# fundamentalvision/BEVFormer

Measured on AMD Instinct MI355X. Metric: BEV-encoder queries/sec (200x200 BEV, 6 cams, 4 lvls), higher is better.
Workload: dtype f32/bf16x3; 1 GPU; bevformer_base BEV encoder forward, 1 frame/step, 200x200 queries, 6 cams, 4 levels, 6 layers, with history BEV; sca_row_order=image, global_batch=1, parallelism=single GPU

## Files before the change

### bevformer_amd/csrc/bevmsda_linear.hip

```cpp
#include "../../include/bevmsda.h"
#include "linear_mfma.h"
#include "linear_pipe.h"
#include "linear_panel.h"
#include "linear_chain.h"
#include "wgrad_mfma.h"
#include "wgrad_tr.h"

namespace {
constexpr bool kLinearPipeDefault = false;
constexpr long long kLinearPipeMaxRows = 8192;
constexpr long long kChainSmallRows = 8192;
inline bool misaligned(const void *p) { return (reinterpret_cast<uintptr_t>(p) & 15u) != 0; }
}

extern "C" {

static int linear_launch(const float *x0, const float *a0, const float *x1, const float *a1, const float *w,
                         const uint16_t *wpack, const float *bias, const bevmsda_linear_desc *d, float *y,
                         void *stream, const int32_t *gidx = nullptr, const float *gscale = nullptr,
                         const float *mask = nullptr, long ldmask = 0, float mask_scale = 1.0f) {
  if (!d) return BEVMSDA_ERR_NULL_POINTER;
  if (d->M < 0 || d->N < 0 || d->K0 < 0 || d->K1 < 0) return BEVMSDA_ERR_BAD_SHAPE;
  if (d->precision != 0 && d->precision != 1) return BEVMSDA_ERR_BAD_OPTION;
  if (d->M == 0 || d->N == 0) return BEVMSDA_OK;
  if (d->K0 == 0 || d->K0 % bevmsda::kLinKGran != 0 || d->K1 % bevmsda::kLinKGran != 0) return BEVMSDA_ERR_UNSUPPORTED;
  if (!x0 || (!w && !wpack) || !y || (d->K1 > 0 && !x1)) return BEVMSDA_ERR_NULL_POINTER;
  if (d->ldx0 % 4 != 0 || (w && d->ldw % 4 != 0) || (a0 && d->lda0 % 4 != 0) ||
      (d->K1 > 0 && (d->ldx1 % 4 != 0 || (a1 && d->lda1 % 4 != 0))))
    return BEVMSDA_ERR_UNSUPPORTED;
  const int gcols = d->group_cols;
  if (gcols < 0) return BEVMSDA_ERR_BAD_SHAPE;
  if (gcols > 0 && (gcols % bevmsda::kLinBN != 0 || d->N % gcols != 0)) return BEVMSDA_ERR_UNSUPPORTED;
  if (d->ldx0 < d->K0 || (w && d->ldw < d->K0 + d->K1) || d->ldy < (gcols > 0 ? gcols : d->N) ||
      (d->K1 > 0 && d->ldx1 < d->K1))
    return BEVMSDA_ERR_BAD_SHAPE;
  if (misaligned(x0) || (w && misaligned(w)) || (wpack && misaligned(wpack)) ||
      (reinterpret_cast<uintptr_t>(y) & 3u) != 0 || (a0 && misaligned(a0)) ||
      (d->K1 > 0 && (misaligned(x1) || (a1 && misaligned(a1)))))
    return BEVMSDA_ERR_MISALIGNED;
  bevmsda::LinArgs a;
  a.x0 = x0; a.a0 = a0; a.x1 = d->K1 > 0 ? x1 : nullptr; a.a1 = d->K1 > 0 ? a1 : nullptr;
  a.ldx0 = d->ldx0; a.lda0 = d->lda0; a.ldx1 = d->ldx1; a.lda1 = d->lda1;
  a.w = w; a.ldw = d->ldw; a.wpack = wpack; a.bias = bias; a.y = y; a.ldy = d->ldy;
  a.gidx = gidx; a.gscale = gscale;
  a.M = d->M; a.N = d->N; a.K0 = d->K0; a.K1 = d->K1; a.relu = d->relu ? 1 : 0;
  a.group_cols = gcols;
  a.out_bf16 = d->out_bf16 ? 1 : 0;
  a.accum = d->reserved[0] == 1 ? 1 : 0;
  if (d->reserved[0] != 0 && d->reserved[0] != 1) return BEVMSDA_ERR_BAD_OPTION;
  a.mask = mask; a.ldmask = ldmask; a.mask_scale = mask_scale;
  if (mask && (gcols != 0 || d->out_bf16 || d->N % 4 != 0 || d->ldy % 4 != 0 || ldmask % 4 != 0 || ldmask < d->N ||
               misaligned(y) || misaligned(mask) || (bias && misaligned(bias)) || d->variant == 131))
    return BEVMSDA_ERR_UNSUPPORTED;
  if (a.accum && (d->out_bf16 || d->N % 4 != 0 || d->ldy % 4 != 0 || gcols % 4 != 0 || misaligned(y) || (bias && misaligned(bias)) ||
                  d->variant == 131))
    return BEVMSDA_ERR_UNSUPPORTED;
  hipStream_t st = static_cast<hipStream_t>(stream);
  const bool add = a.a0 != nullptr || a.a1 != nullptr || gidx != nullptr;
  if (d->variant != 0 && d->variant != 1 && d->variant != 13 && d->variant != 131 && d->variant != 17) return BEVMSDA_ERR_BAD_OPTION;
  if (d->variant == 17) {
    if (!wpack || a.accum || mask || d->N <= 128 || d->N % 4 != 0 || d->ldy % 4 != 0 || misaligned(y) || (bias && misaligned(bias)))
      return BEVMSDA_ERR_UNSUPPORTED;
    const long long nbm = (d->M + 63) / 64, nbn = (d->N + 255) / 256;
    const long long grid = ((nbm + 7) / 8) * 8 * nbn;
    if (grid >= (1LL << 31) || nbm >= (1LL << 28)) return BEVMSDA_ERR_TOO_LARGE;
    a.nblk_m = static_cast<int>(nbm);
    a.nblk_n = static_cast<int>(nbn);
    const dim3 g(static_cast<unsigned>(grid)), b(256);
    if (d->precision == 0) {
      if (add) hipLaunchKernelGGL((bevmsda::linear_splitbf16_kernel<3, true, 32, true, 3, 256, false, 64>), g, b, 0, st, a);
      else hipLaunchKernelGGL((bevmsda::linear_splitbf16_kernel<3, false, 32, true, 3, 256, false, 64>), g, b, 0, st, a);
    } else {
      if (add) hipLaunchKernelGGL((bevmsda::linear_splitbf16_kernel<1, true, 32, true, 3, 256, false, 64>), g, b, 0, st, a);
      else hipLaunchKernelGGL((bevmsda::linear_splitbf16_kernel<1, false, 32, true, 3, 256, false, 64>), g, b, 0, st, a);
    }
    return hipGetLastError() == hipSuccess ? BEVMSDA_OK : BEVMSDA_ERR_LAUNCH;
  }
  {
    const int nch = (d->K0 + d->K1) / 32;
    const bool covered = wpack && !add && !a.accum && !mask && (d->N % 4) == 0 && (d->ldy % 4) == 0 && (gcols % 4) == 0 && !misaligned(y) &&
                         (!bias || !misaligned(bias)) && (!d->out_bf16 || (reinterpret_cast<uintptr_t>(y) & 7u) == 0) &&
                         (nch == 8 || nch == 16);
    if (d->variant == 131 && !covered) return BEVMSDA_ERR_UNSUPPORTED;
    if (covered && (d->variant == 131 || (d->variant == 0 && d->reserved[1] == 0 && (kLinearPipeDefault || d->M <= kLinearPipeMaxRows)))) {
      const long long nbm = (d->M + 127) / 128, nbn = (d->N + 127) / 128;
      const long long grid = ((nbm + 7) / 8) * 8 * nbn;
      if (grid >= (1LL << 31) || nbm >= (1LL << 28)) return BEVMSDA_ERR_TOO_LARGE;
      a.nblk_m = static_cast<int>(nbm);
      a.nblk_n = static_cast<int>(nbn);
#define BEVMSDA_PIPE(NP_, NCH_)                                                                                       \
  do {                                                                                                                \
    auto kern = bevmsda::linear_pipe_kernel<NP_, NCH_>;                                                               \
    const int dyn = 2 * ((NP_) == 3 ? 2 : 1) * bevmsda::kPipePlane * 2;                                               \
    if (hipFuncSetAttribute(reinterpret_cast<const void *>(kern), hipFuncAttributeMaxDynamicSharedMemorySize, dyn) != \
// ... 346 lines not shown
  do {                                                                                                                   \
    if (shape == 1 && deep && (PRE_) == 0)                                                                               \
      hipLaunchKernelGGL((bevmsda::linear_panel_kernel<NP_, 2, 2, 4, LN_, PRE_, 0, 0, false, 6>), grid, dim3(256), 0, st, a); \
    else if (shape == 1) hipLaunchKernelGGL((bevmsda::linear_panel_kernel<NP_, 2, 2, 4, LN_, PRE_>), grid, dim3(256), 0, st, a); \
    else hipLaunchKernelGGL((bevmsda::linear_panel_kernel<NP_, 4, 1, 8, LN_, PRE_>), grid, dim3(512), 0, st, a);           \
  } while (0)
#define BEVMSDA_PANEL(NP_, LN_)                              \
  do {                                                       \
    if (idx) BEVMSDA_PANEL2(NP_, LN_, 2);                    \
    else if (a.a0 || a.a1) BEVMSDA_PANEL2(NP_, LN_, 1);      \
    else BEVMSDA_PANEL2(NP_, LN_, 0);                        \
  } while (0)
  if (d->precision == 0) { if (ln) BEVMSDA_PANEL(3, true); else BEVMSDA_PANEL(3, false); }
  else { if (ln) BEVMSDA_PANEL(1, true); else BEVMSDA_PANEL(1, false); }
#undef BEVMSDA_PANEL2
#undef BEVMSDA_PANEL
  return hipGetLastError() == hipSuccess ? BEVMSDA_OK : BEVMSDA_ERR_LAUNCH;
}

int bevmsda_linear_panel_f32(const float *x0, const float *a0, const float *x1, const float *a1, const int32_t *idx,
                             const float *scale, const uint16_t *wpanel, const float *bias,
                             const bevmsda_linear_desc *d, const bevmsda_layernorm_desc *ln, float *y, void *stream) {
  return panel_launch(x0, a0, x1, a1, idx, scale, wpanel, bias, d, ln, y, stream, nullptr, 0, nullptr, 0);
}

int bevmsda_linear_panel_segments_f32(const float *x0, const uint16_t *wpanel, const float *bias, const bevmsda_linear_desc *d,
                                      const int32_t *seg_start, int64_t seg_len, const int64_t *level_shapes,
                                      int num_levels, float *y, void *stream) {
  if (!seg_start) return BEVMSDA_ERR_NULL_POINTER;
  return panel_launch(x0, nullptr, nullptr, nullptr, nullptr, nullptr, wpanel, bias, d, nullptr, y, stream, seg_start, seg_len,
                      level_shapes, num_levels);
}

int bevmsda_linear_panel_rows2_f32(const float *x_lo, const float *x_hi, int64_t m_split, const uint16_t *wpanel, const float *bias,
                                   const bevmsda_linear_desc *d, float *y, void *stream) {
  if (!x_hi) return BEVMSDA_ERR_NULL_POINTER;
  return panel_launch(x_lo, nullptr, nullptr, nullptr, nullptr, nullptr, wpanel, bias, d, nullptr, y, stream, nullptr, 0, nullptr, 0,
                      x_hi, m_split);
}

struct ChainTail {
  const float *first; long long ld_first;
  const float *pos; long long ld_pos;
  const uint16_t *w3p; const float *b3;
  float *proj; long long ld_proj;
  int n3;
};

static int ffn_chain_launch(const float *rows, const int32_t *idx, const float *scale, const uint16_t *w0p, const float *b0,
                            const float *res, const float *gamma0, const float *beta0, const uint16_t *w1p, const float *b1,
                            const uint16_t *w2p, const float *b2, const float *gamma1, const float *beta1,
                            const bevmsda_chain_desc *d, float *y, void *stream, bool save, float *sv_z0, float *sv_x,
                            float *sv_h, float *sv_z1, const float *dk0 = nullptr, const float *dkh = nullptr,
                            const float *dk1 = nullptr, const ChainTail *tp = nullptr) {
  if (!d) return BEVMSDA_ERR_NULL_POINTER;
  const bool drop = dk0 || dkh || dk1;
  if (tp) {
    if (save || drop) return BEVMSDA_ERR_BAD_OPTION;
    if (tp->n3 <= 0 || tp->n3 > 256 || tp->n3 % 64 != 0) return BEVMSDA_ERR_UNSUPPORTED;
    if (d->M > 0 && (!tp->first || !tp->w3p || !tp->proj)) return BEVMSDA_ERR_NULL_POINTER;
    if (tp->ld_first % 4 != 0 || tp->ld_proj % 4 != 0 || (tp->pos && tp->ld_pos % 4 != 0)) return BEVMSDA_ERR_UNSUPPORTED;
    if (tp->ld_first < 256 || tp->ld_proj < tp->n3 || (tp->pos && tp->ld_pos < 256)) return BEVMSDA_ERR_BAD_SHAPE;
    if (misaligned(tp->first) || misaligned(tp->w3p) || misaligned(tp->proj) || (tp->pos && misaligned(tp->pos)) ||
        (tp->b3 && misaligned(tp->b3)))
      return BEVMSDA_ERR_MISALIGNED;
  }
  if (drop && !save) return BEVMSDA_ERR_BAD_OPTION;
  if ((dk0 && misaligned(dk0)) || (dkh && misaligned(dkh)) || (dk1 && misaligned(dk1))) return BEVMSDA_ERR_MISALIGNED;
  if (save && d->M > 0 && (!sv_z0 || !sv_x || !sv_h || !sv_z1)) return BEVMSDA_ERR_NULL_POINTER;
  if (save && (misaligned(sv_z0) || misaligned(sv_x) || misaligned(sv_h) || misaligned(sv_z1))) return BEVMSDA_ERR_MISALIGNED;
  if (d->M < 0) return BEVMSDA_ERR_BAD_SHAPE;
  if (d->precision != 0 && d->precision != 1) return BEVMSDA_ERR_BAD_OPTION;
  if (d->C != bevmsda::kChainC || d->F != bevmsda::kChainF) return BEVMSDA_ERR_UNSUPPORTED;
  if (d->M == 0) return BEVMSDA_OK;
  if (!rows || !w0p || !w1p || !w2p || !gamma0 || !beta0 || !gamma1 || !beta1 || !y) return BEVMSDA_ERR_NULL_POINTER;
  if ((idx == nullptr) != (scale == nullptr)) return BEVMSDA_ERR_NULL_POINTER;
  if (d->ld_rows % 4 != 0 || d->ld_y % 4 != 0 || (res && d->ld_res % 4 != 0)) return BEVMSDA_ERR_UNSUPPORTED;
  if (d->ld_rows < d->C || d->ld_y < d->C || (res && d->ld_res < d->C)) return BEVMSDA_ERR_BAD_SHAPE;
  if (misaligned(rows) || misaligned(w0p) || misaligned(w1p) || misaligned(w2p) || misaligned(y) || (res && misaligned(res)) ||
      (b0 && misaligned(b0)) || (b1 && misaligned(b1)) || (b2 && misaligned(b2)) || misaligned(gamma0) || misaligned(beta0) ||
      misaligned(gamma1) || misaligned(beta1))
    return BEVMSDA_ERR_MISALIGNED;
  int shape = d->reserved[1];
  if (shape < 0 || shape > 3) return BEVMSDA_ERR_BAD_OPTION;
  const int gst = d->reserved[2] == 0 ? 2 : d->reserved[2];
  if (gst < 2 || gst > 64 || (gst > 2 && (!idx || save))) return BEVMSDA_ERR_BAD_OPTION;
  if (shape == 0) shape = (tp || d->M <= kChainSmallRows) ? 2 : (d->M >= 256LL * 64 ? 2 : 1);
  if (shape == 3) {
    const long long round64 = 256LL * 64;
    const long long head = (d->M / round64) * round64;
    const long long tail = d->M - head;
    if (head == 0 || tail == 0 || tail > 256LL * 2 * 32) {
      bevmsda_chain_desc one = *d;
      one.reserved[1] = (head == 0) ? 2 : 1;
      return ffn_chain_launch(rows, idx, scale, w0p, b0, res, gamma0, beta0, w1p, b1, w2p, b2, gamma1, beta1, &one, y, stream,
                              save, sv_z0, sv_x, sv_h, sv_z1, dk0, dkh, dk1, tp);
    }
    bevmsda_chain_desc dh = *d, dt = *d;
    dh.M = head; dh.reserved[1] = 1;
    dt.M = tail; dt.reserved[1] = 2;
    int rc = ffn_chain_launch(rows, idx, scale, w0p, b0, res, gamma0, beta0, w1p, b1, w2p, b2, gamma1, beta1, &dh, y, stream,
                              save, sv_z0, sv_x, sv_h, sv_z1, dk0, dkh, dk1, tp);
    if (rc != BEVMSDA_OK) return rc;
    const long long o = head;
    ChainTail tt{};
    if (tp) {
      tt = *tp;
      tt.first += o * tp->ld_first;
      if (tt.pos) tt.pos += o * tp->ld_pos;
      tt.proj += o * tp->ld_proj;
    }
    return ffn_chain_launch(idx ? rows : rows + o * d->ld_rows, idx ? idx + o * gst : nullptr, scale ? scale + o : nullptr, w0p, b0,
                            res ? res + o * d->ld_res : nullptr, gamma0, beta0, w1p, b1, w2p, b2, gamma1, beta1, &dt,
                            y + o * d->ld_y, stream, save, save ? sv_z0 + o * 256 : nullptr, save ? sv_x + o * 256 : nullptr,
                            save ? sv_h + o * 512 : nullptr, save ? sv_z1 + o * 256 : nullptr, dk0 ? dk0 + o * 256 : nullptr,
                            dkh ? dkh + o * 512 : nullptr, dk1 ? dk1 + o * 256 : nullptr, tp ? &tt : nullptr);
  }
  const int bm = shape == 1 ? 64 : 32;
  const long long nb = (d->M + bm - 1) / bm;
  if (nb >= (1LL << 31)) return BEVMSDA_ERR_TOO_LARGE;
  bevmsda::ChainArgs a{};
  a.rows = rows; a.ld_rows = d->ld_rows; a.gidx = idx; a.gscale = scale; a.gstride = gst;
  a.w0 = w0p; a.w1 = w1p; a.w2 = w2p; a.b0 = b0; a.b1 = b1; a.b2 = b2;
  a.res = res; a.ld_res = d->ld_res; a.gamma0 = gamma0; a.beta0 = beta0; a.gamma1 = gamma1; a.beta1 = beta1;
  a.eps0 = d->eps0; a.eps1 = d->eps1; a.y = y; a.ld_y = d->ld_y; a.M = d->M;
  a.sv_z0 = sv_z0; a.sv_x = sv_x; a.sv_h = sv_h; a.sv_z1 = sv_z1;
  a.dk0 = dk0; a.dkh = dkh; a.dk1 = dk1;
  if (tp) {
    a.tp_first = tp->first; a.ld_tp_first = tp->ld_first; a.tp_pos = tp->pos; a.ld_tp_pos = tp->ld_pos;
    a.w3 = tp->w3p; a.b3 = tp->b3; a.y3 = tp->proj; a.ld_y3 = tp->ld_proj; a.N3 = tp->n3;
  }
  hipStream_t st = static_cast<hipStream_t>(stream);
  const dim3 grid(static_cast<unsigned>(nb));
#define BEVMSDA_CHAIN_TP(NP_, PRE_)                                                                                               \
  do {                                                                                                                            \
    if (shape == 1) hipLaunchKernelGGL((bevmsda::linear_chain_kernel<NP_, PRE_, 0, 2, 1, 8, false, false, true>), grid, dim3(512), 0, st, a); \
    else hipLaunchKernelGGL((bevmsda::linear_chain_kernel<NP_, PRE_, 0, 1, 2, 4, false, false, true>), grid, dim3(256), 0, st, a);            \
  } while (0)
  if (tp) {
    if (d->precision == 0) { if (idx) BEVMSDA_CHAIN_TP(3, 2); else BEVMSDA_CHAIN_TP(3, 0); }
    else { if (idx) BEVMSDA_CHAIN_TP(1, 2); else BEVMSDA_CHAIN_TP(1, 0); }
    return hipGetLastError() == hipSuccess ? BEVMSDA_OK : BEVMSDA_ERR_LAUNCH;
  }
#undef BEVMSDA_CHAIN_TP
#define BEVMSDA_CHAIN(NP_, PRE_, SV_, DR_)                                                                                        \
  do {                                                                                                                            \
    if (shape == 1) hipLaunchKernelGGL((bevmsda::linear_chain_kernel<NP_, PRE_, 0, 2, 1, 8, SV_, DR_>), grid, dim3(512), 0, st, a); \
    else hipLaunchKernelGGL((bevmsda::linear_chain_kernel<NP_, PRE_, 0, 1, 2, 4, SV_, DR_>), grid, dim3(256), 0, st, a);            \
  } while (0)
  if (drop) {
    if (!idx) return BEVMSDA_ERR_UNSUPPORTED;
    if (d->precision == 0) BEVMSDA_CHAIN(3, 2, true, true); else BEVMSDA_CHAIN(1, 2, true, true);
  } else if (save) {
    if (d->precision == 0) { if (idx) BEVMSDA_CHAIN(3, 2, true, false); else BEVMSDA_CHAIN(3, 0, true, false); }
    else { if (idx) BEVMSDA_CHAIN(1, 2, true, false); else BEVMSDA_CHAIN(1, 0, true, false); }
  } else {
    if (d->precision == 0) { if (idx) BEVMSDA_CHAIN(3, 2, false, false); else BEVMSDA_CHAIN(3, 0, false, false); }
    else { if (idx) BEVMSDA_CHAIN(1, 2, false, false); else BEVMSDA_CHAIN(1, 0, false, false); }
  }
#undef BEVMSDA_CHAIN
  return hipGetLastError() == hipSuccess ? BEVMSDA_OK : BEVMSDA_ERR_LAUNCH;
}

int bevmsda_proj_ffn_chain_f32(const float *rows, const int32_t *idx, const float *scale, const uint16_t *w0p, const float *b0,
                               const float *res, const float *gamma0, const float *beta0, const uint16_t *w1p, const float *b1,
                               const uint16_t *w2p, const float *b2, const float *gamma1, const float *beta1,
                               const bevmsda_chain_desc *d, float *y, void *stream) {
  return ffn_chain_launch(rows, idx, scale, w0p, b0, res, gamma0, beta0, w1p, b1, w2p, b2, gamma1, beta1, d, y, stream, false,
                          nullptr, nullptr, nullptr, nullptr);
}
// ... 32 lines not shown
  if (d->M == 0) return BEVMSDA_OK;
  if (!grad_y || !save_z0 || !save_h || !save_z1 || !gamma0 || !gamma1 || !w0t_p || !w1t_p || !w2t_p || !grad_z1 || !grad_h ||
      !grad_z0 || !grad_in || !grad_gamma_beta1 || !grad_gamma_beta0)
    return BEVMSDA_ERR_NULL_POINTER;
  if (ld_grad_y % 4 != 0) return BEVMSDA_ERR_UNSUPPORTED;
  if (ld_grad_y < d->C) return BEVMSDA_ERR_BAD_SHAPE;
  if (misaligned(grad_y) || misaligned(save_z0) || misaligned(save_h) || misaligned(save_z1) || misaligned(gamma0) ||
      misaligned(gamma1) || misaligned(w0t_p) || misaligned(w1t_p) || misaligned(w2t_p) || misaligned(grad_z1) ||
      misaligned(grad_h) || misaligned(grad_z0) || misaligned(grad_in) || (reinterpret_cast<uintptr_t>(grad_gamma_beta1) & 3u) ||
      (reinterpret_cast<uintptr_t>(grad_gamma_beta0) & 3u))
    return BEVMSDA_ERR_MISALIGNED;
  const long long nb = (d->M + 31) / 32;
  if (nb >= (1LL << 31)) return BEVMSDA_ERR_TOO_LARGE;
  bevmsda::ChainArgs a{};
  a.w0 = w0t_p; a.w1 = w2t_p; a.w2 = w1t_p;
  a.gamma0 = gamma0; a.gamma1 = gamma1; a.eps0 = d->eps0; a.eps1 = d->eps1; a.M = d->M;
  a.bw_gy = grad_y; a.bw_ld_gy = ld_grad_y; a.bw_z1 = save_z1; a.bw_h = save_h; a.bw_z0 = save_z0;
  a.bw_gz1 = grad_z1; a.bw_gh = grad_h; a.bw_gz0 = grad_z0; a.bw_din = grad_in;
  a.bw_dgb1 = grad_gamma_beta1; a.bw_dgb0 = grad_gamma_beta0;
  if (drop0 && !grad_zp) return BEVMSDA_ERR_NULL_POINTER;
  if ((drop0 && misaligned(drop0)) || (drop1 && misaligned(drop1)) || (grad_zp && misaligned(grad_zp))) return BEVMSDA_ERR_MISALIGNED;
  a.dk0 = drop0; a.dk1 = drop1; a.bw_hscale = hidden_scale; a.bw_gzp = grad_zp;
  hipStream_t st = static_cast<hipStream_t>(stream);
  const dim3 grid(static_cast<unsigned>(nb));
  if (d->precision == 0) hipLaunchKernelGGL((bevmsda::linear_chain_kernel<3, 0, 2, 1, 2, 4, false, false>), grid, dim3(256), 0, st, a);
  else hipLaunchKernelGGL((bevmsda::linear_chain_kernel<1, 0, 2, 1, 2, 4, false, false>), grid, dim3(256), 0, st, a);
  return hipGetLastError() == hipSuccess ? BEVMSDA_OK : BEVMSDA_ERR_LAUNCH;
}

int bevmsda_proj_ln_proj_chain_backward_f32(const float *grad_proj, int64_t ld_grad_proj, const float *grad_x, const float *save_z0,
                                            const float *gamma0, const uint16_t *w0t_p, const uint16_t *w1t_p,
                                            const bevmsda_chain_desc *d, float *grad_z0, float *grad_in, float *grad_gamma_beta0,
                                            const float *drop0, float *grad_zp, void *stream) {
  if (!d) return BEVMSDA_ERR_NULL_POINTER;
  if (d->M < 0) return BEVMSDA_ERR_BAD_SHAPE;
  if (d->precision != 0 && d->precision != 1) return BEVMSDA_ERR_BAD_OPTION;
  const int N2 = d->reserved[0];
  if (d->C != bevmsda::kChainC || N2 <= 0 || N2 % 256 != 0 || N2 > bevmsda::kChainMaxN2) return BEVMSDA_ERR_UNSUPPORTED;
  if (d->M == 0) return BEVMSDA_OK;
  if (!grad_proj || !save_z0 || !gamma0 || !w0t_p || !w1t_p || !grad_z0 || !grad_in || !grad_gamma_beta0) return BEVMSDA_ERR_NULL_POINTER;
  if (ld_grad_proj % 4 != 0) return BEVMSDA_ERR_UNSUPPORTED;
  if (ld_grad_proj < N2) return BEVMSDA_ERR_BAD_SHAPE;
  if (misaligned(grad_proj) || (grad_x && misaligned(grad_x)) || misaligned(save_z0) || misaligned(gamma0) || misaligned(w0t_p) ||
      misaligned(w1t_p) || misaligned(grad_z0) || misaligned(grad_in) || (reinterpret_cast<uintptr_t>(grad_gamma_beta0) & 3u))
    return BEVMSDA_ERR_MISALIGNED;
  const long long nb = (d->M + 31) / 32;
  if (nb >= (1LL << 31)) return BEVMSDA_ERR_TOO_LARGE;
  bevmsda::ChainArgs a{};
  a.w0 = w0t_p; a.w1 = w1t_p; a.N2 = N2;
  a.gamma0 = gamma0; a.eps0 = d->eps0; a.M = d->M;
  a.bw_gy = grad_proj; a.bw_ld_gy = ld_grad_proj; a.bw_z1 = grad_x; a.bw_z0 = save_z0;
  a.bw_gz0 = grad_z0; a.bw_din = grad_in; a.bw_dgb0 = grad_gamma_beta0;
  if (drop0 && !grad_zp) return BEVMSDA_ERR_NULL_POINTER;
  if ((drop0 && misaligned(drop0)) || (grad_zp && misaligned(grad_zp))) return BEVMSDA_ERR_MISALIGNED;
  a.dk0 = drop0; a.bw_gzp = grad_zp; a.bw_hscale = 1.f;
  hipStream_t st = static_cast<hipStream_t>(stream);
  const dim3 grid(static_cast<unsigned>(nb));
  if (d->precision == 0) hipLaunchKernelGGL((bevmsda::linear_chain_kernel<3, 0, 3, 1, 2, 4, false, false>), grid, dim3(256), 0, st, a);
  else hipLaunchKernelGGL((bevmsda::linear_chain_kernel<1, 0, 3, 1, 2, 4, false, false>), grid, dim3(256), 0, st, a);
  return hipGetLastError() == hipSuccess ? BEVMSDA_OK : BEVMSDA_ERR_LAUNCH;
}

static int ln_proj_chain_launch(const float *rows, const int32_t *idx, const float *scale, const uint16_t *w0p, const float *b0,
                                const float *res, const float *gamma0, const float *beta0, const uint16_t *w1p, const float *b1,
                                const bevmsda_chain_desc *d, float *x_out, float *proj_out, void *stream, bool save,
                                float *sv_z0, const float *dk0 = nullptr) {
  if (!d) return BEVMSDA_ERR_NULL_POINTER;
  if (dk0 && (!save || misaligned(dk0))) return BEVMSDA_ERR_BAD_OPTION;
  if (save && d->M > 0 && !sv_z0) return BEVMSDA_ERR_NULL_POINTER;
  if (save && misaligned(sv_z0)) return BEVMSDA_ERR_MISALIGNED;
  if (d->M < 0) return BEVMSDA_ERR_BAD_SHAPE;
  if (d->precision != 0 && d->precision != 1) return BEVMSDA_ERR_BAD_OPTION;
  const long ld_y2 = d->reserved[0];
  if (d->C != bevmsda::kChainC || d->F <= 0 || d->F % 32 != 0 || d->F > bevmsda::kChainMaxN2) return BEVMSDA_ERR_UNSUPPORTED;
  if (d->M == 0) return BEVMSDA_OK;
  if (!rows || !w0p || !w1p || !gamma0 || !beta0 || !x_out || !proj_out) return BEVMSDA_ERR_NULL_POINTER;
  if ((idx == nullptr) != (scale == nullptr)) return BEVMSDA_ERR_NULL_POINTER;
  if (d->ld_rows % 4 != 0 || d->ld_y % 4 != 0 || ld_y2 % 4 != 0 || (res && d->ld_res % 4 != 0)) return BEVMSDA_ERR_UNSUPPORTED;
  if (d->ld_rows < d->C || d->ld_y < d->C || ld_y2 < d->F || (res && d->ld_res < d->C)) return BEVMSDA_ERR_BAD_SHAPE;
  if (misaligned(rows) || misaligned(w0p) || misaligned(w1p) || misaligned(x_out) || misaligned(proj_out) || (res && misaligned(res)) ||
      (b0 && misaligned(b0)) || (b1 && misaligned(b1)) || misaligned(gamma0) || misaligned(beta0))
    return BEVMSDA_ERR_MISALIGNED;
  int shape = d->reserved[1];
  if (shape < 0 || shape > 3) return BEVMSDA_ERR_BAD_OPTION;
  if (shape == 0) shape = d->M <= kChainSmallRows ? 2 : (d->M >= 256LL * 64 ? 2 : 1);
  if (d->F % 64 != 0) shape = 1;
  if (shape == 3) {
    const long long round64 = 256LL * 64;
    const long long head = (d->M / round64) * round64;
    const long long tail = d->M - head;
    bevmsda_chain_desc dh = *d, dt = *d;
    if (head == 0 || tail == 0 || tail > 256LL * 2 * 32) {
      dh.reserved[1] = (head == 0) ? 2 : 1;
      return ln_proj_chain_launch(rows, idx, scale, w0p, b0, res, gamma0, beta0, w1p, b1, &dh, x_out, proj_out, stream, save, sv_z0,
                                  dk0);
    }
    dh.M = head; dh.reserved[1] = 1;
    dt.M = tail; dt.reserved[1] = 2;
    int rc = ln_proj_chain_launch(rows, idx, scale, w0p, b0, res, gamma0, beta0, w1p, b1, &dh, x_out, proj_out, stream, save, sv_z0,
                                  dk0);
    if (rc != BEVMSDA_OK) return rc;
    const long long o = head;
    return ln_proj_chain_launch(idx ? rows : rows + o * d->ld_rows, idx ? idx + o * 2 : nullptr, scale ? scale + o : nullptr, w0p,
                                b0, res ? res + o * d->ld_res : nullptr, gamma0, beta0, w1p, b1, &dt, x_out + o * d->ld_y,
                                proj_out + o * ld_y2, stream, save, save ? sv_z0 + o * 256 : nullptr,
                                dk0 ? dk0 + o * 256 : nullptr);
  }
  const int bm = shape == 1 ? 64 : 32;
  const long long nb = (d->M + bm - 1) / bm;
  if (nb >= (1LL << 31)) return BEVMSDA_ERR_TOO_LARGE;
  bevmsda::ChainArgs a{};
  a.rows = rows; a.ld_rows = d->ld_rows; a.gidx = idx; a.gscale = scale;
  a.w0 = w0p; a.w1 = w1p; a.w2 = nullptr; a.b0 = b0; a.b1 = b1; a.b2 = nullptr;
  a.res = res; a.ld_res = d->ld_res; a.gamma0 = gamma0; a.beta0 = beta0; a.gamma1 = a.beta1 = nullptr;
  a.eps0 = d->eps0; a.eps1 = 0.f; a.y = x_out; a.ld_y = d->ld_y; a.M = d->M; a.y2 = proj_out; a.ld_y2 = ld_y2; a.N2 = d->F;
  a.sv_z0 = sv_z0;
  a.dk0 = dk0;
  hipStream_t st = static_cast<hipStream_t>(stream);
  const dim3 grid(static_cast<unsigned>(nb));
#define BEVMSDA_CHAIN(NP_, PRE_, SV_, DR_)                                                                                        \
  do {                                                                                                                            \
    if (shape == 1) hipLaunchKernelGGL((bevmsda::linear_chain_kernel<NP_, PRE_, 1, 2, 1, 8, SV_, DR_>), grid, dim3(512), 0, st, a); \
    else hipLaunchKernelGGL((bevmsda::linear_chain_kernel<NP_, PRE_, 1, 1, 2, 4, SV_, DR_>), grid, dim3(256), 0, st, a);            \
  } while (0)
  if (save) {
    if (idx) return BEVMSDA_ERR_UNSUPPORTED;
    if (dk0) { if (d->precision == 0) BEVMSDA_CHAIN(3, 0, true, true); else BEVMSDA_CHAIN(1, 0, true, true); }
    else { if (d->precision == 0) BEVMSDA_CHAIN(3, 0, true, false); else BEVMSDA_CHAIN(1, 0, true, false); }
  } else {
    if (d->precision == 0) { if (idx) BEVMSDA_CHAIN(3, 2, false, false); else BEVMSDA_CHAIN(3, 0, false, false); }
    else { if (idx) BEVMSDA_CHAIN(1, 2, false, false); else BEVMSDA_CHAIN(1, 0, false, false); }
  }
#undef BEVMSDA_CHAIN
  return hipGetLastError() == hipSuccess ? BEVMSDA_OK : BEVMSDA_ERR_LAUNCH;
}

int bevmsda_proj_ln_proj_chain_f32(const float *rows, const int32_t *idx, const float *scale, const uint16_t *w0p, const float *b0,
                                   const float *res, const float *gamma0, const float *beta0, const uint16_t *w1p, const float *b1,
                                   const bevmsda_chain_desc *d, float *x_out, float *proj_out, void *stream) {
  return ln_proj_chain_launch(rows, idx, scale, w0p, b0, res, gamma0, beta0, w1p, b1, d, x_out, proj_out, stream, false, nullptr);
}

int bevmsda_proj_ln_proj_chain_train_f32(const float *rows, const uint16_t *w0p, const float *b0, const float *res,
                                         const float *gamma0, const float *beta0, const uint16_t *w1p, const float *b1,
                                         const bevmsda_chain_desc *d, float *x_out, float *proj_out, float *save_z0,
                                         const float *drop0, void *stream) {
  return ln_proj_chain_launch(rows, nullptr, nullptr, w0p, b0, res, gamma0, beta0, w1p, b1, d, x_out, proj_out, stream, true,
                              save_z0, drop0);
}

}
```

### bevformer_amd/csrc/linear_chain.h

```cpp
#pragma once
#include <type_traits>
#include "linear_panel.h"
#include "scalar_ops.h"

namespace bevmsda {

struct ChainArgs {
  const float *rows;
  long ld_rows;
  const int32_t *gidx;
  int gstride;
  const float *gscale;
  const uint16_t *w0, *w1, *w2;
  const float *b0, *b1, *b2;
  const float *res;
  long ld_res;
  const float *gamma0, *beta0, *gamma1, *beta1;
  float eps0, eps1;
  float *y;
  long ld_y;
  long M;
  float *y2;
  long ld_y2;
  int N2;
// ... 42 lines not shown

constexpr int kChainC = 256, kChainF = 512;
constexpr int kChainMaxN2 = 768;

template <int NPROD, int PRE, int MODE = 0, int MT = 2, int NT = 1, int NW = 8, bool SAVE = false, bool DROP = false, bool TP = false>
__global__ void __launch_bounds__(NW * 64) __attribute__((amdgpu_waves_per_eu(2, 2)))
linear_chain_kernel(const ChainArgs a) {
  static_assert(NPROD == 1 || NPROD == 3, "NPROD");
  static_assert(!TP || (MODE == 0 && !SAVE && !DROP), "TP: the inference form of MODE 0");
  static_assert(PRE == 0 || PRE == 2, "PRE: 0 plain rows, 2 two-row gather");
  static_assert(MODE < 2 || (MT == 1 && NT == 2 && PRE == 0 && !SAVE && !DROP), "MODE 2 / 3: 32-row workgroups of 4 wavefronts");
  static_assert(NW * NT == 8 && (MT == 1 || MT == 2) && (NT == 1 || NT == 2), "workgroup shape");
  constexpr bool LO = NPROD == 3;
  constexpr int NPL = LO ? 2 : 1;
  constexpr int BM = MT * 32;
  constexpr int NTHREADS = NW * 64;
  constexpr int BUF = (BM / 8) * 4 * 2048;
  constexpr int PPW = (BM / 8) * 4 / NW;
  constexpr int NCST = 4 * kChainC + kChainMaxN2 + 2 * kChainC;
  constexpr int NSTAT = MODE >= 2 ? 2 : 1;
  __shared__ __attribute__((aligned(16))) unsigned char lds[2 * BUF + NSTAT * NW * BM * 4 + NCST * 4];
  unsigned char *const buf0 = lds, *const buf1 = lds + BUF;
  float *const stat = reinterpret_cast<float *>(lds + 2 * BUF);
  float *const cst = stat + NSTAT * NW * BM;
  float *const c_g0 = cst, *const c_be0 = cst + 256, *const c_g1 = cst + 512, *const c_be1 = cst + 768;
  float *const c_b1 = cst + 1024, *const c_b0 = cst + 1024 + kChainMaxN2, *const c_b2 = c_b0 + 256;
  const int nb1 = MODE == 1 ? a.N2 : kChainF;

  const int tid = threadIdx.x;
  const int lane = tid & 63;
  const int wave = __builtin_amdgcn_readfirstlane(tid >> 6);
  const long m0 = static_cast<long>(blockIdx.x) * BM;
#ifdef BEVMSDA_CHAIN_PROF
  unsigned long long t_prev_ = __builtin_readcyclecounter();
#endif

  {
    const float4 z4 = make_float4(0.f, 0.f, 0.f, 0.f);
    for (int t4 = tid * 4; t4 < NCST; t4 += NTHREADS * 4) {
      const float *src = nullptr;
      if (t4 < 256) src = a.gamma0 + t4;
      else if (t4 < 512) src = MODE >= 2 ? nullptr : a.beta0 + (t4 - 256);
      else if (t4 < 768) src = (MODE == 0 || MODE == 2) ? a.gamma1 + (t4 - 512) : nullptr;
      else if (t4 < 1024) src = MODE == 0 ? a.beta1 + (t4 - 768) : nullptr;
      else if (TP && t4 >= 1024 + kChainF && t4 < 1024 + kChainMaxN2)
        src = (a.b3 && t4 - 1024 - kChainF < a.N3) ? a.b3 + (t4 - 1024 - kChainF) : nullptr;
      else if (t4 < 1024 + kChainMaxN2) src = (a.b1 && t4 - 1024 < nb1) ? a.b1 + (t4 - 1024) : nullptr;
      else if (t4 < 1024 + kChainMaxN2 + 256) src = a.b0 ? a.b0 + (t4 - 1024 - kChainMaxN2) : nullptr;
      else src = (MODE == 0 && a.b2) ? a.b2 + (t4 - 1024 - kChainMaxN2 - 256) : nullptr;
      *reinterpret_cast<float4 *>(cst + t4) = src ? *reinterpret_cast<const float4 *>(src) : z4;
    }
  }

  const int f_r = lane & 31, f_h = lane >> 5;
  const int f_q0 = ((f_r >> 2) & 1) | ((f_r >> 4) << 1);
  const int f_rl = ((f_r & 3) << 1) | ((f_r >> 3) & 1);
  const int f_x = f_r & 7;
  unsigned f_addr[4];
#pragma unroll
  for (int sc = 0; sc < 4; ++sc)
    f_addr[sc] = static_cast<unsigned>(f_q0 * 4 * 2048 + (f_rl * 8 + (((2 * sc + f_h) ^ f_x))) * 16);
  unsigned p_addr[NT][4];
#pragma unroll
  for (int j = 0; j < NT; ++j)
#pragma unroll
    for (int g = 0; g < 4; ++g) {
      const int line = NT * wave + j;
      p_addr[j][g] = static_cast<unsigned>((f_q0 * 4 + (line >> 1)) * 2048 + (f_rl * 8 + ((f_h + 2 * g) ^ f_x)) * 16 + (line & 1) * 8);
    }

  const int wlane = lane * 16;
  lin_f32x16 acc[MT][NT], xk[MT][NT], acc2[MODE != 1 ? MT : 1][MODE != 1 ? NT : 1];

#ifndef BEVMSDA_CHAIN_WD
#define BEVMSDA_CHAIN_WD 2
#endif
  constexpr int WD = BEVMSDA_CHAIN_WD;
  lin_bf16x8 wf[WD + 1][NT][NPL];
  auto wload = [&](__amdgpu_buffer_rsrc_t wrsrc, int tile, int nstep, int st, int sg) {
#pragma unroll
    for (int j = 0; j < NT; ++j)
#pragma unroll
      for (int pl = 0; pl < NPL; ++pl)
        wf[st][j][pl] = __builtin_bit_cast(lin_bf16x8, __builtin_amdgcn_raw_buffer_load_b128(
                                                         wrsrc, wlane, (((tile * NT + j) * nstep + sg) * 2 + pl) * 1024, 0));
  };
  auto wprefetch = [&](__amdgpu_buffer_rsrc_t wrsrc, int tile, int nstep, int sg0) {
#pragma unroll
    for (int k = 0; k < WD; ++k) wload(wrsrc, tile, nstep, k, sg0 + k);
  };
  auto gemm16 = [&](auto &c, const unsigned char *buf, __amdgpu_buffer_rsrc_t wrsrc, int tile, int nstep, int sg0) {
    lin_bf16x8 af[2][MT][NPL];
    auto aload = [&](int set, int s) {
      const unsigned base = f_addr[s & 3] + (s >> 2) * 2048;
#pragma unroll
      for (int i = 0; i < MT; ++i)
#pragma unroll
        for (int pl = 0; pl < NPL; ++pl)
          af[set][i][pl] = *reinterpret_cast<const lin_bf16x8 *>(buf + base + i * (4 * 4 * 2048) + pl * 1024);
    };
    aload(0, 0);
#pragma unroll
    for (int s = 0; s < 16; ++s) {
      if (s + WD < 16) wload(wrsrc, tile, nstep, (s + WD) % (WD + 1), sg0 + s + WD);
      if (s + 1 < 16) aload((s + 1) & 1, s + 1);
      __builtin_amdgcn_sched_barrier(0);
#pragma unroll
      for (int j = 0; j < NT; ++j)
#pragma unroll
        for (int i = 0; i < MT; ++i) {
          if constexpr (LO) {
            c[i][j] = __builtin_amdgcn_mfma_f32_32x32x16_bf16(wf[s % (WD + 1)][j][0], af[s & 1][i][1], c[i][j], 0, 0, 0);
            c[i][j] = __builtin_amdgcn_mfma_f32_32x32x16_bf16(wf[s % (WD + 1)][j][1], af[s & 1][i][0], c[i][j], 0, 0, 0);
          }
          c[i][j] = __builtin_amdgcn_mfma_f32_32x32x16_bf16(wf[s % (WD + 1)][j][0], af[s & 1][i][0], c[i][j], 0, 0, 0);
        }
      __builtin_amdgcn_sched_barrier(0);
    }
  };
  auto zero = [&](auto &c) {
#pragma unroll
    for (int i = 0; i < MT; ++i)
#pragma unroll
      for (int j = 0; j < NT; ++j)
#pragma unroll
        for (int r = 0; r < 16; ++r) c[i][j][r] = 0.f;
  };
  auto to_planes = [&](const auto &c, unsigned char *buf) {
#pragma unroll
    for (int i = 0; i < MT; ++i)
#pragma unroll
      for (int j = 0; j < NT; ++j)
#pragma unroll
        for (int g = 0; g < 4; ++g) {
          const float v0 = c[i][j][4 * g], v1 = c[i][j][4 * g + 1], v2 = c[i][j][4 * g + 2], v3 = c[i][j][4 * g + 3];
          uint2 hi, lo;
          hi.x = lin_pack2(v0, v1);
          hi.y = lin_pack2(v2, v3);
          unsigned char *dst = buf + p_addr[j][g] + i * (4 * 4 * 2048);
          *reinterpret_cast<uint2 *>(dst) = hi;
          if (LO) {
            lo.x = lin_pack2(v0 - __uint_as_float(hi.x << 16), v1 - __uint_as_float(hi.x & 0xffff0000u));
            lo.y = lin_pack2(v2 - __uint_as_float(hi.y << 16), v3 - __uint_as_float(hi.y & 0xffff0000u));
            *reinterpret_cast<uint2 *>(dst + 1024) = lo;
          }
        }
  };
  auto ncol = [&](int j) { return (NT * wave + j) * 32 + 4 * (lane >> 5); };
  auto layernorm = [&](auto &c, const float *gamma, const float *beta, float eps) {
    float mean[MT], rstd[MT];
#pragma unroll
    for (int i = 0; i < MT; ++i) {
      float sum = 0.f;
#pragma unroll
      for (int j = 0; j < NT; ++j)
#pragma unroll
        for (int r = 0; r < 16; ++r) sum += c[i][j][r];
      sum += __shfl_xor(sum, 32, 64);
      mean[i] = sum;
    }
    if (lane < 32) {
#pragma unroll
      for (int i = 0; i < MT; ++i) stat[wave * BM + i * 32 + lane] = mean[i];
    }
    __syncthreads();
#pragma unroll
    for (int i = 0; i < MT; ++i) {
      float t = 0.f;
// ... 588 lines not shown
```

Measured before the change: 10.14 million BEV queries/s.

## Add persistent row-streaming chain kernel with LDS-DMA weight ring for LN+proj

Adds a persistent linear_chain_rows kernel, with one block per CU, where each wave owns 16 rows held in registers. Weight chunks stream through a four-stage LDS ring using global_load_lds DMA, so the GEMM+LayerNorm(+FFN) chain runs without re-reading activations. The kernel becomes the default for the LN+projection chain when M is at least 32768 and nothing is saved; the FFN chain uses it only when shape 4 is requested explicitly. The trade-off is that all waves must load the full weight set in every pass and synchronize at a barrier per chunk, which could limit throughput compared with the tiled panel kernels. A debug L2-probe macro is also added to the older chain kernel.

```diff
diff --git a/bevformer_amd/csrc/bevmsda_linear.hip b/bevformer_amd/csrc/bevmsda_linear.hip
--- a/bevformer_amd/csrc/bevmsda_linear.hip
+++ b/bevformer_amd/csrc/bevmsda_linear.hip
@@ -3,6 +3,7 @@
 #include "linear_pipe.h"
 #include "linear_panel.h"
 #include "linear_chain.h"
+#include "linear_chain_rows.h"
 #include "wgrad_mfma.h"
 #include "wgrad_tr.h"
 
@@ -10,6 +11,23 @@
 constexpr bool kLinearPipeDefault = false;
 constexpr long long kLinearPipeMaxRows = 8192;
 constexpr long long kChainSmallRows = 8192;
+constexpr long long kChainRowsMinRows = 32768;
+inline int device_cus() {
+  static int cus[64] = {0};
+  int dev = 0;
+  if (hipGetDevice(&dev) != hipSuccess || dev < 0 || dev >= 64) return 256;
+  if (cus[dev] == 0) {
+    int n = 0;
+    if (hipDeviceGetAttribute(&n, hipDeviceAttributeMultiprocessorCount, dev) != hipSuccess || n <= 0) n = 256;
+    cus[dev] = n;
+  }
+  return cus[dev];
+}
+inline dim3 chain_rows_grid(long long M) {
+  const long long groups8 = ((M + 15) / 16 + 7) / 8;
+  const long long cus = device_cus();
+  return dim3(static_cast<unsigned>(groups8 < cus ? groups8 : cus));
+}
 inline bool misaligned(const void *p) { return (reinterpret_cast<uintptr_t>(p) & 15u) != 0; }
 }
 
@@ -522,10 +540,33 @@
       misaligned(gamma1) || misaligned(beta1))
     return BEVMSDA_ERR_MISALIGNED;
   int shape = d->reserved[1];
-  if (shape < 0 || shape > 3) return BEVMSDA_ERR_BAD_OPTION;
+  if (shape < 0 || shape > 4) return BEVMSDA_ERR_BAD_OPTION;
   const int gst = d->reserved[2] == 0 ? 2 : d->reserved[2];
   if (gst < 2 || gst > 64 || (gst > 2 && (!idx || save))) return BEVMSDA_ERR_BAD_OPTION;
+  if (shape == 4 && (save || drop)) return BEVMSDA_ERR_BAD_OPTION;
   if (shape == 0) shape = (tp || d->M <= kChainSmallRows) ? 2 : (d->M >= 256LL * 64 ? 2 : 1);
+  if (shape == 4) {
+    bevmsda::ChainArgs a{};
+    a.rows = rows; a.ld_rows = d->ld_rows; a.gidx = idx; a.gscale = scale; a.gstride = gst;
+    a.w0 = w0p; a.w1 = w1p; a.w2 = w2p; a.b0 = b0; a.b1 = b1; a.b2 = b2;
+    a.res = res; a.ld_res = d->ld_res; a.gamma0 = gamma0; a.beta0 = beta0; a.gamma1 = gamma1; a.beta1 = beta1;
+    a.eps0 = d->eps0; a.eps1 = d->eps1; a.y = y; a.ld_y = d->ld_y; a.M = d->M;
+    if (tp) {
+      a.tp_first = tp->first; a.ld_tp_first = tp->ld_first; a.tp_pos = tp->pos; a.ld_tp_pos = tp->ld_pos;
+      a.w3 = tp->w3p; a.b3 = tp->b3; a.y3 = tp->proj; a.ld_y3 = tp->ld_proj; a.N3 = tp->n3;
+    }
+    hipStream_t st = static_cast<hipStream_t>(stream);
+    const dim3 grid = chain_rows_grid(d->M);
+#define BEVMSDA_CHAIN_ROWS(NP_, TP_)                                                                                       \
+  do {                                                                                                                     \
+    if (idx) hipLaunchKernelGGL((bevmsda::linear_chain_rows_kernel<NP_, 2, 0, TP_>), grid, dim3(512), 0, st, a);          \
+    else hipLaunchKernelGGL((bevmsda::linear_chain_rows_kernel<NP_, 0, 0, TP_>), grid, dim3(512), 0, st, a);              \
+  } while (0)
+    if (tp) { if (d->precision == 0) BEVMSDA_CHAIN_ROWS(3, true); else BEVMSDA_CHAIN_ROWS(1, true); }
+    else { if (d->precision == 0) BEVMSDA_CHAIN_ROWS(3, false); else BEVMSDA_CHAIN_ROWS(1, false); }
+#undef BEVMSDA_CHAIN_ROWS
+    return hipGetLastError() == hipSuccess ? BEVMSDA_OK : BEVMSDA_ERR_LAUNCH;
+  }
   if (shape == 3) {
     const long long round64 = 256LL * 64;
     const long long head = (d->M / round64) * round64;
@@ -724,7 +765,26 @@
       (b0 && misaligned(b0)) || (b1 && misaligned(b1)) || misaligned(gamma0) || misaligned(beta0))
     return BEVMSDA_ERR_MISALIGNED;
   int shape = d->reserved[1];
-  if (shape < 0 || shape > 3) return BEVMSDA_ERR_BAD_OPTION;
+  if (shape < 0 || shape > 4) return BEVMSDA_ERR_BAD_OPTION;
+  if (shape == 4 && save) return BEVMSDA_ERR_BAD_OPTION;
+  if (shape == 0 && !save && d->M >= kChainRowsMinRows) shape = 4;
+  if (shape == 4) {
+    bevmsda::ChainArgs a{};
+    a.rows = rows; a.ld_rows = d->ld_rows; a.gidx = idx; a.gscale = scale; a.gstride = 2;
+    a.w0 = w0p; a.w1 = w1p; a.b0 = b0; a.b1 = b1;
+    a.res = res; a.ld_res = d->ld_res; a.gamma0 = gamma0; a.beta0 = beta0;
+    a.eps0 = d->eps0; a.y = x_out; a.ld_y = d->ld_y; a.M = d->M; a.y2 = proj_out; a.ld_y2 = ld_y2; a.N2 = d->F;
+    hipStream_t st = static_cast<hipStream_t>(stream);
+    const dim3 grid = chain_rows_grid(d->M);
+    if (d->precision == 0) {
+      if (idx) hipLaunchKernelGGL((bevmsda::linear_chain_rows_kernel<3, 2, 1, false>), grid, dim3(512), 0, st, a);
+      else hipLaunchKernelGGL((bevmsda::linear_chain_rows_kernel<3, 0, 1, false>), grid, dim3(512), 0, st, a);
+    } else {
+      if (idx) hipLaunchKernelGGL((bevmsda::linear_chain_rows_kernel<1, 2, 1, false>), grid, dim3(512), 0, st, a);
+      else hipLaunchKernelGGL((bevmsda::linear_chain_rows_kernel<1, 0, 1, false>), grid, dim3(512), 0, st, a);
+    }
+    return hipGetLastError() == hipSuccess ? BEVMSDA_OK : BEVMSDA_ERR_LAUNCH;
+  }
   if (shape == 0) shape = d->M <= kChainSmallRows ? 2 : (d->M >= 256LL * 64 ? 2 : 1);
   if (d->F % 64 != 0) shape = 1;
   if (shape == 3) {
diff --git a/bevformer_amd/csrc/linear_chain.h b/bevformer_amd/csrc/linear_chain.h
--- a/bevformer_amd/csrc/linear_chain.h
+++ b/bevformer_amd/csrc/linear_chain.h
@@ -148,8 +148,12 @@
     for (int j = 0; j < NT; ++j)
 #pragma unroll
       for (int pl = 0; pl < NPL; ++pl)
+#ifdef BEVMSDA_CHAIN_L2PROBE
+        wf[st][j][pl] = __builtin_bit_cast(lin_bf16x8, __builtin_amdgcn_raw_buffer_load_b128(wrsrc, wlane, pl * 1024 + 0 * (tile + j + nstep + sg), 0));
+#else
         wf[st][j][pl] = __builtin_bit_cast(lin_bf16x8, __builtin_amdgcn_raw_buffer_load_b128(
                                                          wrsrc, wlane, (((tile * NT + j) * nstep + sg) * 2 + pl) * 1024, 0));
+#endif
   };
   auto wprefetch = [&](__amdgpu_buffer_rsrc_t wrsrc, int tile, int nstep, int sg0) {
 #pragma unroll
diff --git a/bevformer_amd/csrc/linear_chain_rows.h b/bevformer_amd/csrc/linear_chain_rows.h
--- /dev/null
+++ b/bevformer_amd/csrc/linear_chain_rows.h
@@ -0,0 +1,361 @@
+#pragma once
+#include "linear_chain.h"
+
+namespace bevmsda {
+
+constexpr int kChainRowsBM = 128;
+typedef float chrows_f32x4 __attribute__((ext_vector_type(4)));
+
+__device__ __forceinline__ void chrows_wait_vm(int n) {
+  switch (n) {
+    case 0: __builtin_amdgcn_s_waitcnt(0x0F70); break;
+    case 1: __builtin_amdgcn_s_waitcnt(0x0F71); break;
+    case 2: __builtin_amdgcn_s_waitcnt(0x0F72); break;
+    case 3: __builtin_amdgcn_s_waitcnt(0x0F73); break;
+    case 4: __builtin_amdgcn_s_waitcnt(0x0F74); break;
+    case 5: __builtin_amdgcn_s_waitcnt(0x0F75); break;
+    case 6: __builtin_amdgcn_s_waitcnt(0x0F76); break;
+    case 7: __builtin_amdgcn_s_waitcnt(0x0F77); break;
+    default: __builtin_amdgcn_s_waitcnt(0x0F78); break;
+  }
+}
+
+__device__ __forceinline__ void chrows_dma16(const void *src, unsigned lds_dst) {
+  asm volatile("s_mov_b32 m0, %1\n\ts_nop 0\n\tglobal_load_lds_dwordx4 %0, off" : : "v"(src), "s"(lds_dst) : "memory", "m0");
+}
+
+template <int NPROD, int PRE, int MODE, bool TP>
+__global__ void __launch_bounds__(512) __attribute__((amdgpu_waves_per_eu(2, 2)))
+linear_chain_rows_kernel(const ChainArgs a) {
+  static_assert(NPROD == 1 || NPROD == 3, "NPROD");
+  static_assert(PRE == 0 || PRE == 2, "PRE: 0 plain rows, 2 gather");
+  static_assert(MODE == 0 || (MODE == 1 && !TP), "MODE 0 (+ TP) or MODE 1");
+  constexpr bool LO = NPROD == 3;
+  constexpr int NPL = LO ? 2 : 1;
+  constexpr int UB = NPL * 1024;
+  constexpr int PB = 2 * UB;
+  constexpr int CHB = 8 * PB;
+  constexpr int NST = 4;
+  constexpr int NCST = 4 * kChainC + kChainMaxN2 + 2 * kChainC;
+  __shared__ __attribute__((aligned(16))) unsigned char ring[NST * CHB];
+  __shared__ __attribute__((aligned(16))) float cst[NCST];
+  float *const c_g0 = cst, *const c_be0 = cst + 256, *const c_g1 = cst + 512, *const c_be1 = cst + 768;
+  float *const c_b1 = cst + 1024, *const c_b0 = cst + 1024 + kChainMaxN2, *const c_b2 = c_b0 + 256;
+  const int nb1 = MODE == 1 ? a.N2 : kChainF;
+
+  const int tid = threadIdx.x;
+  const int lane = tid & 63;
+  const int wave = __builtin_amdgcn_readfirstlane(tid >> 6);
+  const int fr = lane & 15, fh = lane >> 4;
+  const int nt3 = TP ? a.N3 / 32 : 0;
+  const int nchunk = MODE == 1 ? 8 + a.N2 / 32 : 8 + 32 + (TP ? 16 : 0);
+
+  const long ngroup = (a.M + 15) / 16;
+  const long gb = ngroup * blockIdx.x / gridDim.x, ge = ngroup * (blockIdx.x + 1) / gridDim.x;
+  const int npass = static_cast<int>((ge - gb + 7) / 8);
+  const int total = npass * nchunk;
+
+  struct Chunk { const unsigned char *img; int u0, ustr, np; };
+  auto chunk_of = [&](int c) __attribute__((always_inline)) -> Chunk {
+    if (c < 8) return {reinterpret_cast<const unsigned char *>(a.w0), 2 * c, 16, 8};
+    c -= 8;
+    if (MODE == 1) return {reinterpret_cast<const unsigned char *>(a.w1), 16 * c, 2, 8};
+    if (c < 32) {
+      const int G = c >> 2, k = c & 3;
+      if (k < 2) return {reinterpret_cast<const unsigned char *>(a.w1), 16 * (2 * G + k), 2, 8};
+      return {reinterpret_cast<const unsigned char *>(a.w2), 4 * G + 2 * (k - 2), 32, 8};
+    }
+    c -= 32;
+    return {reinterpret_cast<const unsigned char *>(a.w3), c < 8 ? 16 + 2 * c : 2 * (c - 8), 32, nt3};
+  };
+  const unsigned ring_base = static_cast<unsigned>(reinterpret_cast<size_t>((__attribute__((address_space(3))) unsigned char *)ring));
+  auto dma = [&](int gc) __attribute__((always_inline)) {
+    const Chunk k = chunk_of(gc % nchunk);
+    if (wave >= k.np) return;
+    const unsigned char *src = k.img + static_cast<long>(k.u0 + k.ustr * wave) * 2048 + lane * 16;
+    const unsigned dst = __builtin_amdgcn_readfirstlane(ring_base + (gc & (NST - 1)) * CHB + wave * PB);
+#pragma unroll
+    for (int u = 0; u < 2; ++u)
+#pragma unroll
+      for (int pl = 0; pl < NPL; ++pl) chrows_dma16(src + (u * 2 + pl) * 1024, dst + u * UB + pl * 1024);
+  };
+  auto chunk_wait = [&](int gc) __attribute__((always_inline)) -> const unsigned char * {
+    int n = 0;
+#pragma unroll
+    for (int k = 1; k <= NST - 2; ++k)
+      if (gc + k < total && wave < chunk_of((gc + k) % nchunk).np) n += 2 * NPL;
+    chrows_wait_vm(n);
+    asm volatile("s_waitcnt lgkmcnt(0)\n\ts_barrier" ::: "memory");
+    if (gc + NST - 1 < total) dma(gc + NST - 1);
+    return ring + (gc & (NST - 1)) * CHB;
+  };
+
+  {
+    const float4 z4 = make_float4(0.f, 0.f, 0.f, 0.f);
+    for (int t4 = tid * 4; t4 < NCST; t4 += 512 * 4) {
+      const float *src = nullptr;
+      if (t4 < 256) src = a.gamma0 + t4;
+      else if (t4 < 512) src = a.beta0 + (t4 - 256);
+      else if (t4 < 768) src = MODE == 0 ? a.gamma1 + (t4 - 512) : nullptr;
+      else if (t4 < 1024) src = MODE == 0 ? a.beta1 + (t4 - 768) : nullptr;
+      else if (TP && t4 >= 1024 + kChainF && t4 < 1024 + kChainMaxN2)
+        src = (a.b3 && t4 - 1024 - kChainF < a.N3) ? a.b3 + (t4 - 1024 - kChainF) : nullptr;
+      else if (t4 < 1024 + kChainMaxN2) src = (a.b1 && t4 - 1024 < nb1) ? a.b1 + (t4 - 1024) : nullptr;
+      else if (t4 < 1024 + kChainMaxN2 + 256) src = a.b0 ? a.b0 + (t4 - 1024 - kChainMaxN2) : nullptr;
+      else src = (MODE == 0 && a.b2) ? a.b2 + (t4 - 1024 - kChainMaxN2 - 256) : nullptr;
+      *reinterpret_cast<float4 *>(cst + t4) = src ? *reinterpret_cast<const float4 *>(src) : z4;
+    }
+  }
+#pragma unroll
+  for (int c = 0; c < NST - 2; ++c)
+    if (c < total) dma(c);
+  if (NST - 2 < total) dma(NST - 2);
+
+  const unsigned fro0 = static_cast<unsigned>((fh >> 1) * UB + (fr + 32 * (fh & 1)) * 16);
+  auto mma = [&](chrows_f32x4 &c, const unsigned char *slot, int pc, int half, const lin_bf16x8 &xh, const lin_bf16x8 &xl)
+      __attribute__((always_inline)) {
+    const unsigned char *p = slot + pc * PB + fro0 + half * 256;
+    const lin_bf16x8 wh = *reinterpret_cast<const lin_bf16x8 *>(p);
+    if constexpr (LO) {
+      const lin_bf16x8 wl = *reinterpret_cast<const lin_bf16x8 *>(p + 1024);
+      c = __builtin_amdgcn_mfma_f32_16x16x32_bf16(wh, xl, c, 0, 0, 0);
+      c = __builtin_amdgcn_mfma_f32_16x16x32_bf16(wl, xh, c, 0, 0, 0);
+    }
+    c = __builtin_amdgcn_mfma_f32_16x16x32_bf16(wh, xh, c, 0, 0, 0);
+  };
+  auto split = [&](const chrows_f32x4 &p, const chrows_f32x4 &q, lin_bf16x8 &h, lin_bf16x8 &l) __attribute__((always_inline)) {
+    uint4 hi, lo;
+    lin_split8<LO>(make_float4(p[0], p[1], p[2], p[3]), make_float4(q[0], q[1], q[2], q[3]), hi, lo);
+    h = __builtin_bit_cast(lin_bf16x8, hi);
+    if (LO) l = __builtin_bit_cast(lin_bf16x8, lo);
+  };
+  auto f4 = [](const float4 &v) __attribute__((always_inline)) { return chrows_f32x4{v.x, v.y, v.z, v.w}; };
+  auto ld4 = [](const float *p) __attribute__((always_inline)) { return *reinterpret_cast<const float4 *>(p); };
+
+  lin_bf16x8 xh[8], xl[8];
+  chrows_f32x4 v[16];
+  auto to_frags = [&]() __attribute__((always_inline)) {
+#pragma unroll
+    for (int s = 0; s < 8; ++s) split(v[4 * (s >> 1) + (s & 1)], v[4 * (s >> 1) + (s & 1) + 2], xh[s], xl[s]);
+  };
+  auto layernorm = [&](const float *gamma, const float *beta, float eps) __attribute__((always_inline)) {
+    float sum = 0.f;
+#pragma unroll
+    for (int t = 0; t < 16; ++t)
+#pragma unroll
+      for (int e = 0; e < 4; ++e) sum += v[t][e];
+    sum += __shfl_xor(sum, 16, 64);
+    sum += __shfl_xor(sum, 32, 64);
+    const float mean = sum * (1.0f / kChainC);
+    float ss = 0.f;
+#pragma unroll
+    for (int t = 0; t < 16; ++t)
+#pragma unroll
+      for (int e = 0; e < 4; ++e) {
+        const float d = v[t][e] - mean;
+        ss = fmaf(d, d, ss);
+      }
+    ss += __shfl_xor(ss, 16, 64);
+    ss += __shfl_xor(ss, 32, 64);
+    const float rstd = rsqrtf(fma_scalar(ss, 1.0f / kChainC, eps));
+#pragma unroll
+    for (int t = 0; t < 16; ++t) {
+      const float4 ga = ld4(gamma + 16 * t + 4 * fh), be = ld4(beta + 16 * t + 4 * fh);
+      v[t][0] = (v[t][0] - mean) * rstd * ga.x + be.x;
+      v[t][1] = (v[t][1] - mean) * rstd * ga.y + be.y;
+      v[t][2] = (v[t][2] - mean) * rstd * ga.z + be.z;
+      v[t][3] = (v[t][3] - mean) * rstd * ga.w + be.w;
+    }
+  };
+
+#pragma unroll 1
+  for (int pass = 0; pass < npass; ++pass) {
+    const long g = gb + pass * 8 + wave;
+    const bool active = g < ge;
+    const long mrow = g * 16 + fr;
+    const bool mok = active && mrow < a.M;
+    const long mclamp = mrow < a.M ? mrow : a.M - 1;
+    const int c0 = pass * nchunk;
+    auto store_rows = [&](float *out, long ld) __attribute__((always_inline)) {
+      if (!mok) return;
+      float *yrow = out + mrow * ld + 4 * fh;
+#pragma unroll
+      for (int t = 0; t < 16; ++t)
+        *reinterpret_cast<float4 *>(yrow + 16 * t) = make_float4(v[t][0], v[t][1], v[t][2], v[t][3]);
+    };
+
+    if (active) {
+      float4 q[16];
+      if (PRE == 2) {
+        const int gst = a.gstride > 2 ? a.gstride : 2;
+        const int g0 = a.gidx[mclamp * gst], g1 = a.gidx[mclamp * gst + 1];
+        const float gs = a.gscale[mclamp];
+        const float *r0 = a.rows + static_cast<long>(g0 < 0 ? 0 : g0) * a.ld_rows + 4 * fh;
+        const float *r1 = a.rows + static_cast<long>(g1 < 0 ? 0 : g1) * a.ld_rows + 4 * fh;
+#pragma unroll
+        for (int t = 0; t < 16; ++t) q[t] = ld4(r0 + 16 * t);
+        if (gst > 2 && a.gidx[mclamp * gst + 2] >= 0) {
+          for (int j = 2; j < gst; ++j) {
+            const int r = a.gidx[mclamp * gst + j];
+            if (r < 0) break;
+            const float *rx = a.rows + static_cast<long>(r) * a.ld_rows + 4 * fh;
+#pragma unroll
+            for (int t = 0; t < 16; ++t) q[t] = lin_add4(q[t], ld4(rx + 16 * t));
+          }
+        }
+#pragma unroll
+        for (int t = 0; t < 16; ++t) q[t] = panel_gsum(q[t], g0 >= 0, ld4(r1 + 16 * t), g1 >= 0, gs);
+      } else {
+        const float *r0 = a.rows + mclamp * a.ld_rows + 4 * fh;
+#pragma unroll
+        for (int t = 0; t < 16; ++t) q[t] = ld4(r0 + 16 * t);
+      }
+#pragma unroll
+      for (int s = 0; s < 8; ++s) split(f4(q[4 * (s >> 1) + (s & 1)]), f4(q[4 * (s >> 1) + (s & 1) + 2]), xh[s], xl[s]);
+      if (a.res) {
+        const float *rr = a.res + mclamp * a.ld_res + 4 * fh;
+#pragma unroll
+        for (int t = 0; t < 16; ++t) v[t] = f4(ld4(rr + 16 * t));
+      } else {
+#pragma unroll
+        for (int t = 0; t < 16; ++t) v[t] = chrows_f32x4{0.f, 0.f, 0.f, 0.f};
+      }
+    }
+
+#pragma unroll
+    for (int s = 0; s < 8; ++s) {
+      const unsigned char *slot = chunk_wait(c0 + s);
+      if (active) {
+#pragma unroll
+        for (int T = 0; T < 8; ++T)
+#pragma unroll
+          for (int half = 0; half < 2; ++half) mma(v[2 * T + half], slot, T, half, xh[s], xl[s]);
+      }
+    }
+    if (active) {
+#pragma unroll
+      for (int t = 0; t < 16; ++t) v[t] += f4(ld4(c_b0 + 16 * t + 4 * fh));
+      layernorm(c_g0, c_be0, a.eps0);
+      if constexpr (MODE == 1) store_rows(a.y, a.ld_y);
+      to_frags();
+    }
+
+    if constexpr (MODE == 1) {
+      const int ntile = a.N2 / 32;
+#pragma unroll 1
+      for (int T = 0; T < ntile; ++T) {
+        const unsigned char *slot = chunk_wait(c0 + 8 + T);
+        if (active) {
+          chrows_f32x4 p[2];
+#pragma unroll
+          for (int half = 0; half < 2; ++half) p[half] = f4(ld4(c_b1 + 32 * T + 16 * half + 4 * fh));
+#pragma unroll
+          for (int s = 0; s < 8; ++s)
+#pragma unroll
+            for (int half = 0; half < 2; ++half) mma(p[half], slot, s, half, xh[s], xl[s]);
+          if (mok) {
+            float *prow = a.y2 + mrow * a.ld_y2 + 32 * T + 4 * fh;
+#pragma unroll
+            for (int half = 0; half < 2; ++half)
+              *reinterpret_cast<float4 *>(prow + 16 * half) = make_float4(p[half][0], p[half][1], p[half][2], p[half][3]);
+          }
+        }
+      }
+    } else {
+      if (active) {
+#pragma unroll
+        for (int t = 0; t < 16; ++t) v[t] += f4(ld4(c_b2 + 16 * t + 4 * fh));
+      }
+#pragma unroll 1
+      for (int G = 0; G < 8; ++G) {
+        const int cg = c0 + 8 + 4 * G;
+        chrows_f32x4 hacc[4];
+        lin_bf16x8 hh[2], hl[2];
+#pragma unroll
+        for (int k = 0; k < 2; ++k) {
+          const unsigned char *slot = chunk_wait(cg + k);
+          if (active) {
+#pragma unroll
+            for (int half = 0; half < 2; ++half) hacc[2 * k + half] = f4(ld4(c_b1 + 16 * (4 * G + 2 * k + half) + 4 * fh));
+#pragma unroll
+            for (int s = 0; s < 8; ++s)
+#pragma unroll
+              for (int half = 0; half < 2; ++half) mma(hacc[2 * k + half], slot, s, half, xh[s], xl[s]);
+          }
+        }
+        if (active) {
+#pragma unroll
+          for (int i = 0; i < 4; ++i)
+#pragma unroll
+            for (int e = 0; e < 4; ++e) hacc[i][e] = hacc[i][e] < 0.f ? 0.f : hacc[i][e];
+#pragma unroll
+          for (int u = 0; u < 2; ++u) split(hacc[u], hacc[u + 2], hh[u], hl[u]);
+        }
+#pragma unroll
+        for (int u = 0; u < 2; ++u) {
+          const unsigned char *slot = chunk_wait(cg + 2 + u);
+          if (active) {
+#pragma unroll
+            for (int T = 0; T < 8; ++T)
+#pragma unroll
+              for (int half = 0; half < 2; ++half) mma(v[2 * T + half], slot, T, half, hh[u], hl[u]);
+          }
+        }
+      }
+      if (active) {
+        layernorm(c_g1, c_be1, a.eps1);
+        store_rows(a.y, a.ld_y);
+      }
+      if constexpr (TP) {
+        if (active) {
+          if (a.tp_pos) {
+            const float *pr = a.tp_pos + mclamp * a.ld_tp_pos + 4 * fh;
+#pragma unroll
+            for (int t = 0; t < 16; ++t) v[t] += f4(ld4(pr + 16 * t));
+          }
+          to_frags();
+#pragma unroll
+          for (int t = 0; t < 16; ++t) v[t] = f4(ld4(c_b1 + kChainF + 16 * t + 4 * fh));
+        }
+#pragma unroll
+        for (int s = 0; s < 8; ++s) {
+          const unsigned char *slot = chunk_wait(c0 + 40 + s);
+          if (active) {
+#pragma unroll
+            for (int T = 0; T < 8; ++T)
+              if (T < nt3) {
+#pragma unroll
+                for (int half = 0; half < 2; ++half) mma(v[2 * T + half], slot, T, half, xh[s], xl[s]);
+              }
+          }
+        }
+        if (active) {
+          const float *fp = a.tp_first + mclamp * a.ld_tp_first + 4 * fh;
+#pragma unroll
+          for (int s = 0; s < 8; ++s)
+            split(f4(ld4(fp + 16 * (4 * (s >> 1) + (s & 1)))), f4(ld4(fp + 16 * (4 * (s >> 1) + (s & 1) + 2))), xh[s], xl[s]);
+        }
+#pragma unroll
+        for (int s = 0; s < 8; ++s) {
+          const unsigned char *slot = chunk_wait(c0 + 48 + s);
+          if (active) {
+#pragma unroll
+            for (int T = 0; T < 8; ++T)
+              if (T < nt3) {
+#pragma unroll
+                for (int half = 0; half < 2; ++half) mma(v[2 * T + half], slot, T, half, xh[s], xl[s]);
+              }
+          }
+        }
+        if (mok) {
+          float *prow = a.y3 + mrow * a.ld_y3 + 4 * fh;
+#pragma unroll
+          for (int t = 0; t < 16; ++t)
+            if (t < 2 * nt3) *reinterpret_cast<float4 *>(prow + 16 * t) = make_float4(v[t][0], v[t][1], v[t][2], v[t][3]);
+        }
+      }
+    }
+  }
+}
+
+}
```

After: 10.24 million BEV queries/s (median of 6 runs). No clear change (+0.9%).
